# HyeontaeSung/CC-MPC

Measured on AMD Instinct MI355X. Metric: MPC constraint-gen cycles/sec @20Hz (np=5000, ph=8); ellipsoid ΔF-norm vs ref, higher is better.
Workload: dtype f64; 1 GPU; C2: 1 scene x 4 OVs, np=5000/OV, ph=8, Minkowski/MVOE constraint-gen cycle (moments + all (cell,t,tau) half-spaces), one ccmpc_minkowski_cycle launch per step, particles resident in HBM; scenes_per_gpu=1, O=4, N_per_ov=5000, T=8, cells=9, halfspaces_per_cycle=252

## Files before the change

### cc-mpc_amd/csrc/constraints.hpp

```cpp
#pragma once
#include "ccmpc_common.hpp"

namespace ccmpc {


struct M2 {
  double a, b, c, d;
};

__device__ __forceinline__ M2 mul(const M2 &x, const M2 &y) {
  return {x.a * y.a + x.b * y.c, x.a * y.b + x.b * y.d, x.c * y.a + x.d * y.c,
          x.c * y.b + x.d * y.d};
}
__device__ __forceinline__ M2 scale(const M2 &x, double s) {
  return {x.a * s, x.b * s, x.c * s, x.d * s};
}
__device__ __forceinline__ M2 sub(const M2 &x, const M2 &y) {
  return {x.a - y.a, x.b - y.b, x.c - y.c, x.d - y.d};
}
__device__ __forceinline__ M2 add(const M2 &x, const M2 &y) {
  return {x.a + y.a, x.b + y.b, x.c + y.c, x.d + y.d};
}
__device__ __forceinline__ M2 transpose(const M2 &x) { return {x.a, x.c, x.b, x.d}; }

// ... 158 lines not shown
  static constexpr uint64_t start_word() {
    uint64_t x = 0;
    for (int t = 1; t < TC && t < 8; ++t) x |= static_cast<uint64_t>(t * (t - 1) / 2) << (8 * t);
    return x;
  }
};
template <int TC>
__device__ __forceinline__ void pair_of_tc(int p, int &t, int &tau) {
  if constexpr (PairTable<TC>::kFits) {
    constexpr uint64_t lo = PairTable<TC>::t_word(0), hi = PairTable<TC>::t_word(1);
    constexpr uint64_t start = PairTable<TC>::start_word();
    t = static_cast<int>(((p < 16 ? lo : hi) >> (4 * (p & 15))) & 15);
    tau = p - static_cast<int>((start >> (8 * t)) & 255);
  } else {
    pair_of(p, t, tau);
  }
}


static_assert(sizeof(ccmpc_halfspace) == 128, "record size");
static_assert(offsetof(ccmpc_halfspace, d) == 16 && offsetof(ccmpc_halfspace, q01) == 32 &&
                  offsetof(ccmpc_halfspace, r00) == 48 && offsetof(ccmpc_halfspace, r11) == 64 &&
                  offsetof(ccmpc_halfspace, mean0) == 96 && offsetof(ccmpc_halfspace, which) == 112,
              "16-byte field pairs of ccmpc_halfspace");
__device__ __forceinline__ void store_pair(double *p, double a, double b) {
  *reinterpret_cast<double2 *>(p) = make_double2(a, b);
}

struct MinkParams {
  const double *ref_traj;
  const int32_t *cell_ref;
  const double *cell_risk;
  double R, tol;
  int maxiter;
  ccmpc_halfspace *out_rec;
  double *out_prob_lower;
};

struct PairMoments {
  M2 c_t, cov_mu, cov_infer;
  bool ok;
};

struct BlockInverse {
  M2 inv;
  bool ok;
};
__device__ __forceinline__ BlockInverse block_inverse(const M2 &c_tau) {
  BlockInverse bi;
  bi.ok = inv2(c_tau, bi.inv);
  return bi;
}

__device__ __forceinline__ PairMoments pair_moments(const double *C, int rows, int t, int tau) {
  PairMoments pm;
  const BlockInverse bi = block_inverse(block(C, rows, tau, tau));
  pm.c_t = block(C, rows, t, t);
  const M2 c_x = block(C, rows, t, tau);
  const M2 c_xT = block(C, rows, tau, t);
  pm.ok = bi.ok;
  pm.cov_mu = mul(mul(c_x, bi.inv), c_xT);
  pm.cov_infer = sub(pm.c_t, pm.cov_mu);
  return pm;
}

__device__ __forceinline__ double pair_lower_bound(const PairMoments &pm, double gamma) {
  const double root_t = sqrt(fro(pm.c_t));
  const double al = sqrt(fro(pm.cov_infer)) / root_t;
  const double be = sqrt(fro(pm.cov_mu)) / root_t;
  const double x = gamma * (1.0 - al) / be;
  return -expm1(-0.5 * (x * x));
}

__device__ __forceinline__ double pair_scale(const PairMoments &pm, double chi_p, double gamma) {
  const double root_t = sqrt(fro(pm.c_t));
  const double alpha = sqrt(fro(pm.cov_infer)) / root_t;
  const double beta = sqrt(fro(pm.cov_mu)) / root_t;
  const double x = sqrt(chi_p) * beta / gamma + alpha;
  return x * x;
}

__device__ __forceinline__ int closest_tangent(const M2 &S, double c, double n0, double n1,
                                               double proj, double nrm, double na, double &d,
                                               int &which) {
  const double sn0 = S.a * n0 + S.b * n1, sn1 = S.c * n0 + S.d * n1;
  const double q = n0 * sn0 + n1 * sn1;
  if (q <= 0.0) {
    d = NAN;
    which = 0;
    return CCMPC_REC_NO_TANGENT;
  }
  const double delta = c * sqrt(q);
  const double d1 = proj + delta, d2 = proj - delta;
  const double dist0 = fabs(na - d1) / nrm, dist1 = fabs(na - d2) / nrm;
  which = (dist1 < dist0) ? 1 : 0;
  d = which ? d2 : d1;
  return 0;
}

struct TangentFrame {
  double m, n0, proj, nrm, na;
};
__device__ __forceinline__ TangentFrame tangent_frame(double m0, double m1, double a0, double a1) {
  TangentFrame f;
  f.m = -(a0 - m0) / (a1 - m1);
  f.n0 = -f.m;
  const double n1 = 1.0;
  f.proj = f.n0 * m0 + n1 * m1;
  f.nrm = sqrt(f.n0 * f.n0 + n1 * n1);
  f.na = f.n0 * a0 + n1 * a1;
  return f;
}

template <int TC = 0>
__device__ void minkowski_pair(const double *C, const double *mu, const double *ref, int rows_arg,
                               int t, int tau, double chi_r, double chi_p, double R, double tol,
                               int maxiter, ccmpc_halfspace *out) {
  const int rows = TC ? 2 * TC : rows_arg;
  const double m0 = mu[2 * t], m1 = mu[2 * t + 1];
  const TangentFrame f = tangent_frame(m0, m1, ref[2 * t], ref[2 * t + 1]);
  const double m = f.m, n0 = f.n0, n1 = 1.0, proj = f.proj, nrm = f.nrm, na = f.na;
  store_pair(&out->n0, n0, n1);
  store_pair(&out->mean0, m0, m1);
  const PairMoments pm = pair_moments(C, rows, t, tau);
  int status = 0;
  double b1 = NAN, b2 = NAN;
  M2 Q = {NAN, NAN, NAN, NAN}, QR = {NAN, NAN, NAN, NAN};
  bool ok = compute_mvoe(scale(pm.cov_infer, chi_r), scale(pm.cov_mu, chi_p), tol, maxiter, b1, Q,
                         pm.ok);
  store_pair(&out->q01, Q.b, Q.d);
  ok = compute_mvoe(Q, M2{R * R, 0.0, 0.0, R * R}, tol, maxiter, b2, QR, ok);
  if (!ok) status = CCMPC_REC_SINGULAR;
  store_pair(&out->r00, QR.a, QR.b);
  store_pair(&out->r11, QR.d, b1);
  out->beta2 = b2;
  double d = NAN;
  int which = 0, side = 0;
  if (!isfinite(m)) {
    if (status == 0) status = CCMPC_REC_NONFINITE;
  } else {
    const int ts = closest_tangent(QR, 1.0, n0, n1, proj, nrm, na, d, which);
    if (ts != 0) {
      if (status == 0) status = ts;
    } else if (isfinite(d)) {
      side = (proj <= d) ? 1 : -1;
    }
  }
  if (status == 0 && !(isfinite(d) && isfinite(Q.a) && isfinite(QR.a) && isfinite(m0)))
    status = CCMPC_REC_NONFINITE;
  store_pair(&out->d, d, Q.a);
  *reinterpret_cast<int4 *>(&out->which) = make_int4(which, side, status, (t << 16) | tau);
}

template <int NTH, int TC = 0>
__device__ void minkowski_cell(const double *C, const double *mu, int T_arg, int cell,
                               const double *ref, double chi_r, double chi_p, double gamma,
                               const MinkParams &mp, double *lb_s, int tid) {
  constexpr int nthreads = NTH;
  const int T = TC ? TC : T_arg;
  const int rows = 2 * T;
  const int P = T * (T - 1) / 2;
  ccmpc_halfspace *rec = mp.out_rec + static_cast<int64_t>(cell) * P;
  const int half = (nthreads >= 128 && P <= nthreads / 2) ? nthreads / 2 : 0;
  if (half && P <= 2 * 64) {
    if (tid < half) {
      if (tid < P) {
        int t, tau;
        pair_of_tc<TC>(tid, t, tau);
        minkowski_pair<TC>(C, mu, ref, rows, t, tau, chi_r, chi_p, mp.R, mp.tol, mp.maxiter,
                           rec + tid);
      }
      return;
    }
    const int lane = tid - half;
    if (lane >= 64) return;
    for (int p = lane; p < P; p += 64) {
      int t, tau;
      pair_of_tc<TC>(p, t, tau);
      const double lb = pair_lower_bound(pair_moments(C, rows, t, tau), gamma);
      lb_s[p] = lb;
      rec[p].lower_bound = lb;
    }
    asm volatile("s_waitcnt lgkmcnt(0)" ::: "memory");
    if (lane < T) {
      double v = 1.0;
      for (int tau = 0; tau < lane; ++tau) v = fmin(v, lb_s[lane * (lane - 1) / 2 + tau]);
      mp.out_prob_lower[static_cast<int64_t>(cell) * T + lane] = v;
    }
    return;
  }
  const bool lb_side = half && tid >= half;
  const int base = lb_side ? tid - half : tid, stride = half ? half : nthreads;
  for (int p = base; p < P; p += stride) {
    int t, tau;
    pair_of_tc<TC>(p, t, tau);
    if (lb_side || !half) {
      const double lb = pair_lower_bound(pair_moments(C, rows, t, tau), gamma);
      lb_s[p] = lb;
      rec[p].lower_bound = lb;
    }
    if (!lb_side)
      minkowski_pair<TC>(C, mu, ref, rows, t, tau, chi_r, chi_p, mp.R, mp.tol, mp.maxiter, rec + p);
  }
  __syncthreads();
  for (int t = tid; t < T; t += nthreads) {
    double v = 1.0;
    for (int tau = 0; tau < t; ++tau) v = fmin(v, lb_s[t * (t - 1) / 2 + tau]);
    mp.out_prob_lower[static_cast<int64_t>(cell) * T + t] = v;
  }
}

template <int NTH>
__device__ void minkowski_cell(const double *C, const double *mu, int T, int cell,
                               const MinkParams &mp, double *lb_s, int tid) {
  const int rsel = mp.cell_ref ? mp.cell_ref[cell] : 0;
  const double *ref = mp.ref_traj + static_cast<int64_t>(rsel) * (2 * T);
  minkowski_cell<NTH>(C, mu, T, cell, ref, mp.cell_risk[3 * cell + 0],
                      mp.cell_risk[3 * cell + 1], mp.cell_risk[3 * cell + 2], mp, lb_s, tid);
}

void launch_minkowski_rows(const double *mean, const double *cov, int T, int n_cells,
                           const MinkParams &mp, hipStream_t s);

}
```

### cc-mpc_amd/csrc/moments.hip

```cpp
#include "ccmpc_common.hpp"

#ifndef CCMPC_PROBE
#define CCMPC_PROBE 0
#endif

#if CCMPC_PROBE & 4
constexpr int kProbeSlots = 8, kProbeMaxWG = 8192;
__device__ unsigned long long g_probe_ts[kProbeMaxWG * kProbeSlots];
__device__ unsigned long long g_probe_stream_end[kProbeMaxWG];
__device__ __forceinline__ unsigned long long &probe_stream_end_lds() {
  __shared__ unsigned long long t;
  return t;
}
#define PROBE_STREAM_END()                                                                     \
  do {                                                                                         \
    if ((threadIdx.x & 63) == 0)                                                               \
      atomicMax(&probe_stream_end_lds(), __builtin_amdgcn_s_memrealtime());                    \
  } while (0)
#define PROBE_TS(k)                                                                            \
  do {                                                                                         \
    if (threadIdx.x == 0 && blockIdx.x < kProbeMaxWG)                                          \
      g_probe_ts[blockIdx.x * kProbeSlots + (k)] = __builtin_amdgcn_s_memrealtime();           \
    if ((k) == 0 && !(CCMPC_PROBE & 16) && threadIdx.x == 0 && blockIdx.x < kProbeMaxWG)       \
      g_probe_ts[blockIdx.x * kProbeSlots + 7] =                                               \
// ... 115 lines not shown
struct LaneVec<P, 4> {
  using type = Quad<P>;
  __device__ static void load(const P *p, type &q) { load_quad(p, q); }
};
template <typename P>
struct LaneVec<P, 2> {
  using type = Pair<P>;
  __device__ static void load(const P *p, type &q) { load_pair(p, q); }
};

template <typename P, int RB, int S, int W>
__device__ __forceinline__ void load_group(typename LaneVec<P, W>::type (&v)[S][RB],
                                           const P *const (&rowp)[RB], int64_t gbase, int64_t p1,
                                           int g) {
  const int64_t qlast = (p1 - 1) & ~int64_t(W - 1);
#pragma unroll
  for (int s = 0; s < S; ++s) {
    const int64_t q = gbase + 4 * W * s + W * g;
    const int64_t qc = q < qlast ? q : qlast;
#pragma unroll
    for (int b = 0; b < RB; ++b) {
#if CCMPC_PROBE & 2
      LaneVec<P, W>::load(rowp[b] + (qc & (W - 1)), v[s][b]);
#else
      LaneVec<P, W>::load(rowp[b] + qc, v[s][b]);
#endif
    }
  }
}

#ifndef CCMPC_SUBSTEP_FENCE
#define CCMPC_SUBSTEP_FENCE 1
#endif
__device__ __forceinline__ void pin_loaded(Quad<double> &q) {
  ccmpc_d2v lo = {q.lo.x, q.lo.y}, hi = {q.hi.x, q.hi.y};
  asm volatile("" : "+v"(lo), "+v"(hi));
  q.lo = make_double2(lo.x, lo.y);
  q.hi = make_double2(hi.x, hi.y);
}
__device__ __forceinline__ void pin_loaded(Quad<float> &q) {
  ccmpc_f4v t = {q.v.x, q.v.y, q.v.z, q.v.w};
  asm volatile("" : "+v"(t));
  q.v = make_float4(t.x, t.y, t.z, t.w);
}
template <typename P>
__device__ __forceinline__ void pin_loaded(Pair<P> &) {}
template <typename P, int RB, int S, int NACC, int W>
__device__ __forceinline__ void mfma_group(const typename LaneVec<P, W>::type (&raw)[S][RB],
                                           const double (&sh)[RB], const bool (&live)[RB],
                                           int64_t gbase, int64_t p1, int g,
                                           d4 (&acc)[NACC][n_tiles(RB)], double (&s1)[RB]) {
#pragma unroll
  for (int s = 0; s < S; ++s) {
    const int64_t q = gbase + 4 * W * s + W * g;
    typename LaneVec<P, W>::type x[RB];
#pragma unroll
    for (int b = 0; b < RB; ++b) x[b] = raw[s][b];
#if CCMPC_SUBSTEP_FENCE
    if (S > 1) {
      __builtin_amdgcn_sched_barrier(0);
#pragma unroll
      for (int b = 0; b < RB; ++b) pin_loaded(x[b]);
    }
#endif
    double v[RB][W];
#pragma unroll
    for (int b = 0; b < RB; ++b)
#pragma unroll
      for (int j = 0; j < W; ++j)
#if CCMPC_PROBE & 32
        v[b][j] = x[b][j] - sh[b];
#elif CCMPC_PROBE & 64
        v[b][j] = x[b][j];
#else
        v[b][j] = (live[b] && q + j < p1) ? x[b][j] - sh[b] : 0.0;
#endif
#pragma unroll
    for (int j = 0; j < W; ++j) {
      const int a = (NACC == 2) ? (j & 1) : 0;
      int t = 0;
#pragma unroll
      for (int bi = 0; bi < RB; ++bi)
#pragma unroll
        for (int bj = bi; bj < RB; ++bj) {
#if CCMPC_PROBE & 1
          acc[a][t][0] += v[bi][j] * v[bj][j];
#else
          acc[a][t] = __builtin_amdgcn_mfma_f64_16x16x4f64(v[bi][j], v[bj][j], acc[a][t], 0, 0, 0);
#endif
          ++t;
        }
    }
#pragma unroll
    for (int b = 0; b < RB; ++b)
      s1[b] += W == 4 ? (v[b][0] + v[b][1]) + (v[b][2 % W] + v[b][3 % W]) : v[b][0] + v[b][1];
  }
}

#ifndef CCMPC_DEFER_ROOT
#define CCMPC_DEFER_ROOT 1
#endif
__host__ __device__ constexpr bool defer_root(int rb, bool mink, bool bal) {
  return CCMPC_DEFER_ROOT && bal && !mink && rb >= 4;
}

struct EpilogueLds {
  double *slab, *shift, *S, *mean, *cov, *lb, *ref;
  int *flag;
};

#ifndef CCMPC_TAIL_LANDED
#define CCMPC_TAIL_LANDED 1
#endif
template <typename Sch, int NTH, bool MINK, bool COV_IN_LDS, bool DEFER, int TC = 0,
          typename Publish>
__device__ __forceinline__ void cell_epilogue(Publish publish, const ItemLoc &loc, int32_t nit,
                                              int T_arg, const TreeLayout &tree,
                                              const double *__restrict__ origin,
                                              double *__restrict__ out_mean,
                                              double *__restrict__ out_cov, const MinkParams &mp,
                                              const EpilogueLds &L) {
  constexpr int E = Sch::E;
  constexpr bool kLastOrder = std::is_same<Sch, Scheme16<1>>::value;
  const int T = TC ? TC : T_arg;
  const int cell = loc.cell, rows = 2 * T;
  const double o0 = origin ? origin[2 * cell] : 0.0, o1 = origin ? origin[2 * cell + 1] : 0.0;
  double *mean = out_mean + static_cast<int64_t>(cell) * rows;
  double *cov = out_cov + static_cast<int64_t>(cell) * rows * rows;
  if (nit == 1) {
    publish(L.slab, true);
    PROBE_TS(3);
    PROBE_TS(4);
  } else {
    publish(tree.slabs[0] + static_cast<int64_t>(loc.first + loc.chunk_idx) * E, false);
    PROBE_TS(3);
    if (DEFER && nit <= kRootFanIn) return;
    const double *root;
    int32_t root_n;
    const bool last = tree_climb<E, NTH>(tree, loc.chunk_idx, nit, loc.first, cell, L.flag,
                                         &root, &root_n);
    PROBE_TS(4);
    if (!last) return;
    gather_root<Sch, NTH, TC, kLastOrder && CCMPC_GATHER_ORDERED != 0>(
        root, root_n, rows, L.slab, L.cov);
    PROBE_GATHERED();
  }
  if (kLastOrder && CCMPC_TAIL_LANDED != 0 && MINK)
    __builtin_amdgcn_s_waitcnt(0x0f70);
  finalize_cell<Sch, NTH, TC>([&](int e) { return double2{L.slab[e], L.slab[e + 1]}; }, loc.cnt,
                              T, L.shift, L.S, o0, o1, mean, cov, L.mean,
                              COV_IN_LDS ? L.cov : nullptr, L.slab + Sch::GRAM);
  PROBE_TS(5);
  if (MINK)
    minkowski_cell<NTH, TC>(COV_IN_LDS ? L.cov : cov, L.mean, T, cell, L.ref, L.ref[rows],
                            L.ref[rows + 1], L.ref[rows + 2], mp, L.lb, threadIdx.x);
  PROBE_TS(6);
}

struct WaveRange {
  int64_t p0, stride, p1, ngroups;
};
template <bool BAL>
__device__ __forceinline__ WaveRange wave_range(int64_t a, int64_t b, int w, int nw, int64_t wq,
                                                int64_t gs) {
  WaveRange r;
  if (BAL) {
    r.p0 = a + static_cast<int64_t>(w) * gs;
    r.stride = nw * gs;
    r.p1 = b;
    r.ngroups = r.p0 < b ? ceil_div(b - r.p0, r.stride) : 0;
  } else {
    r.p0 = a + static_cast<int64_t>(w) * wq;
    r.stride = gs;
    r.p1 = (r.p0 + wq < b) ? r.p0 + wq : b;
    r.ngroups = r.p1 > r.p0 ? ceil_div(r.p1 - r.p0, gs) : 0;
  }
  return r;
}

#ifndef CCMPC_TAIL_LATE
#define CCMPC_TAIL_LATE 1
#endif
__device__ __forceinline__ double prefetch_tail(const MinkParams &mp, const ItemLoc &loc,
                                                int rows) {
#if CCMPC_TAIL_LATE
  const int i = min(static_cast<int>(threadIdx.x), rows + 2);
  const bool ref = i < rows;
  const double *base = ref ? mp.ref_traj : mp.cell_risk;
  const int64_t at =
      ref ? static_cast<int64_t>(loc.ref_sel) * rows + i : int64_t(3 * loc.cell + (i - rows));
  return base[at];
#else
  if (threadIdx.x < rows) return mp.ref_traj[static_cast<int64_t>(loc.ref_sel) * rows + threadIdx.x];
  if (threadIdx.x < rows + 3) return mp.cell_risk[3 * loc.cell + (threadIdx.x - rows)];
  return 0.0;
#endif
}
__device__ __forceinline__ double prefetch_tail_landed(const MinkParams &mp, const ItemLoc &loc,
                                                       int rows) {
  const double v = prefetch_tail(mp, loc, rows);
  __builtin_amdgcn_sched_barrier(0);
  __builtin_amdgcn_s_waitcnt(0x0f70);
  return v;
}

#ifndef CCMPC_T_CONST
#define CCMPC_T_CONST 1
#endif
#ifndef CCMPC_LOCATE_STRAIGHT
#define CCMPC_LOCATE_STRAIGHT 1
#endif
#ifndef CCMPC_SLOT_FRONT
#define CCMPC_SLOT_FRONT 1
#endif
using SlotArg = uint64_t;
inline SlotArg slot_arg(int64_t slot_cap, int64_t ips) {
  const uint64_t magic = (uint64_t(1) << 31) / static_cast<uint64_t>(ips) + 1u;
  return static_cast<uint64_t>(static_cast<uint32_t>(slot_cap)) | (magic << 32);
}
template <bool SLOT>
using OffArg = std::conditional_t<SLOT, SlotArg, const int64_t *__restrict__>;
#ifndef CCMPC_LOADS_FIRST
#define CCMPC_LOADS_FIRST 1
#endif
template <typename P, int RB, bool MINK, bool BAL, int TC = 0, bool SLOT = false>
__global__ __launch_bounds__(Geo<RB>::THREADS,
                             (MINK && RB == 1) ? 3 : Geo<RB>::MIN_WAVES_PER_SIMD)
void moments_kernel(
    const int64_t *__restrict__ cell_cnt, OffArg<SLOT> cell_off,
    const int32_t *__restrict__ cell_ref, const P *__restrict__ pos, int64_t ld, int n_cells,
    int lg_wq, int32_t whole32, int T_arg, const double *__restrict__ origin, TreeLayout tree,
    double *__restrict__ out_mean, double *__restrict__ out_cov, MinkParams mp) {
  using G = Geo<RB>;
  static_assert(TC == 0 || 2 * TC == 16 * RB, "a constant horizon fills its row blocks exactly");
  const int T = TC ? TC : T_arg;
  const int64_t whole = whole32;
  constexpr int NT = n_tiles(RB);
  constexpr int NACC = G::NACC;
  constexpr int D = 16 * RB;
  constexpr int S = G::S;
  constexpr int W = RB >= 4 ? kWBig : 4;
  constexpr int E = slab_doubles(RB);
  constexpr bool COV_IN_LDS = MINK;
  constexpr bool DEFER = defer_root(RB, MINK, BAL);
  constexpr int XCH = combine_xch_doubles(RB, G::NW) > (MINK ? D * D : 0)
                          ? combine_xch_doubles(RB, G::NW) : D * D;
  static_assert(XCH >= gather_part_doubles(E), "xch must hold the root gather's group slabs");
  __shared__ double xch[XCH];
  __shared__ double slab_lds[E];
  __shared__ double shift_lds[D];
  __shared__ double S_lds[D];
  __shared__ double mean_lds[D];
  __shared__ double lb_s[MINK ? 40 * 39 / 2 : 1];
  __shared__ double ref_lds[MINK ? D + 3 : 1];
  __shared__ int flag;

  const int lane = threadIdx.x & 63;
  const int w = __builtin_amdgcn_readfirstlane(threadIdx.x >> 6);
  const int rows = 2 * T;
  const int lg_chunk = lg_wq + lg_waves_per_item(RB);

  auto item = [=](const ItemLoc &loc_in, int32_t nit, int64_t a, int64_t b) {
    const int r = lane & 15;
    const int g = lane >> 4;
    ItemLoc loc = loc_in;
    int64_t cnt = loc.cnt;
    double pre = (MINK && !CCMPC_TAIL_LATE) ? prefetch_tail(mp, loc, rows) : 0.0;
    constexpr int DP = RB >= 3 ? CCMPC_DEPTH_BIG : kDepth;
    constexpr bool FRONT = CCMPC_LOADS_FIRST != 0 && RB == 1 && !BAL;
    double sh[RB];
    d4 acc[NACC][NT];
    double s1[RB];
    if constexpr (FRONT) {
      constexpr int GS = 4 * W * S;
      static_assert(RB == 1 && GS == 64, "the front is written for RB = 1");
      bool rr = b - a > (int64_t(1) << lg_chunk);
      int64_t p0 = a + (rr ? int64_t(w) * GS : int64_t(w) << lg_wq);
      const bool live0 = r < rows;
      int64_t row_at = static_cast<int64_t>(live0 ? r : 0) * ld + loc.off;
      const P *rowp[RB];
      bool live[RB] = {live0};
      typename LaneVec<P, W>::type buf[DP][S][RB];
      int64_t p1, ngroups, st;
      double x0s = 0.0;
      if constexpr (SLOT) {
        const int64_t p0s =
            (static_cast<int64_t>(loc.chunk_idx) << lg_chunk) + (int64_t(w) << lg_wq);
        const int64_t n_ld = cell_cnt[loc.cell];
        __builtin_amdgcn_sched_barrier(0);
        x0s = static_cast<double>(pos[row_at]);
        const P *gb = pos + (row_at + p0s);
#pragma unroll
        for (int s = 0; s < S; ++s) {
#if CCMPC_PROBE & 2
          LaneVec<P, W>::load(pos + row_at + ((W * g) & (W - 1)), buf[0][s][0]);
#else
          LaneVec<P, W>::load(gb + (4 * W * s + W * g), buf[0][s][0]);
#endif
        }
        asm volatile("" ::: "memory");
        __builtin_amdgcn_sched_barrier(0);
        const int32_t *rp = cell_ref ? cell_ref + loc.cell
                                     : reinterpret_cast<const int32_t *>(cell_cnt + loc.cell);
        const int32_t rs_ld = *rp;
        PROBE_TS(1);
        cnt = n_ld;
        loc.cnt = n_ld;
        loc.ref_sel = cell_ref ? rs_ld : 0;
// ... 179 lines not shown
      __builtin_expect(static_cast<unsigned>(n_cells - 1) < 64u, 1)) {
    if (!locate_item_straight(blockIdx.x, cell_cnt, cell_off, n_cells, lg_chunk, loc, cell_ref,
                              whole))
      return;
  } else {
    if (!locate_item(blockIdx.x, cell_cnt, cell_off, n_cells, lg_chunk, loc,
                     cell_ref, whole))
      return;
    if (CCMPC_LOCATE_STRAIGHT != 0 && RB == 1) __builtin_amdgcn_s_waitcnt(0x0f70);
  }
  PROBE_TS(1);
  const int32_t nit = items_of(loc.cnt, lg_chunk, whole);
  const int64_t i0 = static_cast<int64_t>(loc.chunk_idx) << lg_chunk;
  const int64_t i1 = nit == 1 ? loc.cnt : min(i0 + (int64_t(1) << lg_chunk), loc.cnt);
  item(loc, nit, i0, i1);
  }
}

#ifndef CCMPC_F32_WIDE4
#define CCMPC_F32_WIDE4 1
#endif
template <typename P>
struct Row4 {
  using type = Pair<P>;
  static constexpr int W = 2;
  __device__ static void load(const P *p, type &q) { load_pair(p, q); }
};
#if CCMPC_F32_WIDE4
template <>
struct Row4<float> {
  using type = Quad<float>;
  static constexpr int W = 4;
  __device__ static void load(const float *p, type &q) {
    if constexpr (CCMPC_NT_PAIR != 0) {
      const ccmpc_f4v t = __builtin_nontemporal_load(reinterpret_cast<const ccmpc_f4v *>(p));
      q.v = make_float4(t.x, t.y, t.z, t.w);
    } else {
      q.v = *reinterpret_cast<const float4 *>(p);
    }
  }
};
#endif

template <typename P, int NB>
__device__ __forceinline__ void load_group4(typename Row4<P>::type (&v)[NB],
                                            const P *const (&rowp)[NB], int64_t gbase, int64_t p1,
                                            int m) {
  constexpr int W = Row4<P>::W;
  const int64_t qlast = (p1 - 1) & ~int64_t(W - 1);
  const int64_t q = gbase + W * m;
  const int64_t qc = q < qlast ? q : qlast;
#pragma unroll
  for (int I = 0; I < NB; ++I) Row4<P>::load(rowp[I] + qc, v[I]);
}

#ifndef CCMPC_ROWLOAD4
#define CCMPC_ROWLOAD4 0
#endif
__device__ __forceinline__ double bperm_f64(int addr, double x) {
  const uint64_t u = __builtin_bit_cast(uint64_t, x);
  const uint32_t lo = static_cast<uint32_t>(
      __builtin_amdgcn_ds_bpermute(addr, static_cast<int>(static_cast<uint32_t>(u))));
  const uint32_t hi = static_cast<uint32_t>(
      __builtin_amdgcn_ds_bpermute(addr, static_cast<int>(static_cast<uint32_t>(u >> 32))));
  return __builtin_bit_cast(double, (static_cast<uint64_t>(hi) << 32) | lo);
}
__device__ __forceinline__ float bperm_f32(int addr, float x) {
  return __builtin_bit_cast(
      float, __builtin_amdgcn_ds_bpermute(addr, __builtin_bit_cast(int, x)));
}
__device__ __forceinline__ Pair<double> bperm_pair(int addr, const Pair<double> &p) {
  Pair<double> r;
  r.v.x = bperm_f64(addr, p.v.x);
  r.v.y = bperm_f64(addr, p.v.y);
  return r;
}
__device__ __forceinline__ Pair<float> bperm_pair(int addr, const Pair<float> &p) {
  Pair<float> r;
  r.v.x = bperm_f32(addr, p.v.x);
  r.v.y = bperm_f32(addr, p.v.y);
  return r;
}

template <typename P, int NB>
__device__ __forceinline__ void mfma_group4(const typename Row4<P>::type (&loaded)[NB],
                                            const double (&sh)[NB], const bool (&live)[NB],
                                            int64_t gbase, int64_t p1, int m, int paddr,
                                            double (&acc)[n_pairs(NB)], double (&s1)[NB]) {
  constexpr int W = Row4<P>::W;
  const int64_t q = gbase + W * m;
#if CCMPC_ROWLOAD4
  static_assert(W == 2, "CCMPC_ROWLOAD4 is the pair layout");
  Pair<P> raw[NB];
#pragma unroll
  for (int I = 0; I < NB; ++I) raw[I] = bperm_pair(paddr, loaded[I]);
#else
  const typename Row4<P>::type(&raw)[NB] = loaded;
  (void)paddr;
#endif
#pragma unroll
  for (int j = 0; j < W; ++j) {
    double v[NB];
#pragma unroll
    for (int I = 0; I < NB; ++I) {
#if CCMPC_PROBE & 32
      v[I] = raw[I][j] - sh[I];
#elif CCMPC_PROBE & 64
      v[I] = raw[I][j];
#else
      v[I] = (live[I] && q + j < p1) ? raw[I][j] - sh[I] : 0.0;
#endif
      s1[I] += v[I];
    }
    int p = 0;
#pragma unroll
    for (int I = 0; I < NB; ++I)
#pragma unroll
      for (int J = I; J < NB; ++J) {
        acc[p] = __builtin_amdgcn_mfma_f64_4x4x4f64(v[I], v[J], acc[p], 0, 0, 0);
        ++p;
      }
  }
}

#ifndef CCMPC_NW4
#define CCMPC_NW4 4
#endif
constexpr int kNW4 = CCMPC_NW4;
constexpr int kThreads4 = kNW4 * 64;
#ifndef CCMPC_M4_OCC
#define CCMPC_M4_OCC(NB) (((NB) <= 5 ? 3 : 2) * 4 / kNW4 > 0 ? ((NB) <= 5 ? 3 : 2) * 4 / kNW4 : 1)
#endif
#ifndef CCMPC_M4_OCC_F32
#define CCMPC_M4_OCC_F32 0
#endif
template <typename P>
constexpr int m4_occ(int nb) {
  return std::is_same_v<P, float> && CCMPC_M4_OCC_F32 > 0 ? CCMPC_M4_OCC_F32 : CCMPC_M4_OCC(nb);
}

template <typename P, int NB, bool MINK, bool BAL>
__global__ __launch_bounds__(kThreads4, m4_occ<P>(NB)) void moments4_kernel(
    const int64_t *__restrict__ cell_cnt, const int64_t *__restrict__ cell_off,
    const int32_t *__restrict__ cell_ref, const P *__restrict__ pos, int64_t ld, int n_cells,
    int lg_wq, int T, const double *__restrict__ origin, TreeLayout tree,
    double *__restrict__ out_mean, double *__restrict__ out_cov, MinkParams mp) {
  using Sch = Scheme4<NB>;
  constexpr int NP = Sch::NP, D = Sch::D, E = Sch::E;
  __shared__ double xch[kNW4 * Combine4Layout<NB>::XS];
  __shared__ double slab_lds[E];
  __shared__ double shift_lds[D];
  __shared__ double S_lds[D];
  __shared__ double mean_lds[D];
  __shared__ double lb_s[MINK ? 12 * 11 / 2 : 1];
  __shared__ double ref_lds[MINK ? D + 3 : 1];
  __shared__ int flag;

  const int lane = threadIdx.x & 63;
  const int w = __builtin_amdgcn_readfirstlane(threadIdx.x >> 6);
  const int rows = 2 * T;
  const int lg_chunk = lg_wq + 2;

  auto item = [=](const ItemLoc &loc, int32_t nit, int64_t a, int64_t b) {
    const int c = lane & 3, m = lane >> 2;
#if CCMPC_ROWLOAD4
    const int rl = lane >> 4, ml = lane & 15;
#else
    const int rl = c, ml = m;
#endif
    const int paddr = 4 * (16 * c + m);
    const int64_t cnt = loc.cnt;
    double pre = (MINK && !CCMPC_TAIL_LATE) ? prefetch_tail(mp, loc, rows) : 0.0;
    const WaveRange wr = wave_range<BAL>(a, b, w, kNW4, int64_t(1) << lg_wq, 16 * Row4<P>::W);
    const int64_t p1 = wr.p1;

    double sh[NB];
    const P *rowp[NB];
    bool live[NB];
#pragma unroll
    for (int I = 0; I < NB; ++I) {
      const int R = 4 * I + c, RL = 4 * I + rl;
      live[I] = R < rows;
      rowp[I] = pos + static_cast<int64_t>(RL < rows ? RL : 0) * ld + loc.off;
      sh[I] = (live[I] && cnt > 0)
                  ? static_cast<double>(pos[static_cast<int64_t>(R) * ld + loc.off]) : 0.0;
    }
    double acc[NP];
#pragma unroll
    for (int p = 0; p < NP; ++p) acc[p] = 0.0;
    double s1[NB];
#pragma unroll
    for (int I = 0; I < NB; ++I) s1[I] = 0.0;

    const int64_t ngroups = wr.ngroups, st = wr.stride;
    constexpr int DP = BAL ? (std::is_same_v<P, float> ? kDepth4BalF32 : kDepth4Bal) : kDepth4;
    typename Row4<P>::type buf[DP][NB];
    if (ngroups > 0) {
#pragma unroll
      for (int d = 0; d < DP - 1; ++d) load_group4<P, NB>(buf[d], rowp, wr.p0 + d * st, p1, ml);
      if (MINK && CCMPC_TAIL_LATE) {
        __builtin_amdgcn_sched_barrier(0);
        pre = prefetch_tail(mp, loc, rows);
      }
      int64_t gi = 0;
      for (; gi + DP <= ngroups; gi += DP) {
        if (BAL) progress_prio(gi, ngroups);
#pragma unroll
        for (int d = 0; d < DP; ++d) {
          load_group4<P, NB>(buf[(d + DP - 1) % DP], rowp, wr.p0 + (gi + d + DP - 1) * st, p1, ml);
          __builtin_amdgcn_sched_barrier(0);
          mfma_group4<P, NB>(buf[d], sh, live, wr.p0 + (gi + d) * st, p1, m, paddr, acc, s1);
          __builtin_amdgcn_sched_barrier(0);
        }
      }
#pragma unroll
      for (int d = 0; d < DP - 1; ++d)
        if (gi + d < ngroups)
          mfma_group4<P, NB>(buf[d], sh, live, wr.p0 + (gi + d) * st, p1, m, paddr, acc, s1);
    } else if (MINK && CCMPC_TAIL_LATE) {
      pre = prefetch_tail_landed(mp, loc, rows);
    }
    PROBE_TS(2);
    PROBE_STREAM_END();
#if CCMPC_PROGRESS_PRIO
    __builtin_amdgcn_s_setprio(0);
#endif

    if (MINK && threadIdx.x < rows + 3) ref_lds[threadIdx.x] = pre;
#pragma unroll
    for (int I = 0; I < NB; ++I)
      if (w == 0 && m == 0) shift_lds[4 * I + c] = sh[I];
    static_assert(kNW4 * Combine4Layout<NB>::XS >= D * D, "xch must hold the covariance");
    static_assert(kNW4 * Combine4Layout<NB>::XS >= gather_part_doubles(E),
                  "xch must hold the root gather's group slabs");
    const EpilogueLds L{slab_lds, shift_lds, S_lds, mean_lds, xch, lb_s, ref_lds, &flag};
    cell_epilogue<Sch, kThreads4, MINK, MINK, false>(
        [&](double *dst, bool to_lds) { combine4<NB, kNW4>(acc, s1, xch, dst, to_lds); }, loc,
        nit, T, tree, origin, out_mean, out_cov, mp, L);
  };

  PROBE_TS(0);
  if (BAL) {
    ItemLoc loc;
    int64_t chunk;
    if (!locate_balanced(blockIdx.x, gridDim.x, cell_cnt, cell_off, n_cells, loc, &chunk,
                         cell_ref))
      return;
    PROBE_TS(1);
    const int64_t i0 = static_cast<int64_t>(loc.chunk_idx) * chunk;
    item(loc, static_cast<int32_t>(loc.cnt > 0 ? ceil_div_fast(loc.cnt, chunk) : 1), i0,
         min(i0 + chunk, loc.cnt));
    return;
  }
  ItemLoc loc;
  if (!locate_item(blockIdx.x, cell_cnt, cell_off, n_cells, lg_chunk, loc,
                   cell_ref))
    return;
  PROBE_TS(1);
  const int64_t i0 = static_cast<int64_t>(loc.chunk_idx) << lg_chunk;
  const int64_t i1 = min(i0 + (int64_t(1) << lg_chunk), loc.cnt);
  item(loc, items_of(loc.cnt, lg_chunk), i0, i1);
}

__device__ __forceinline__ void cell_items_balanced(int cell, int G, const int64_t *__restrict__ cnt,
                                                    int n_cells, int32_t &first, int32_t &nit,
                                                    int64_t &n) {
  const int lane = threadIdx.x & 63;
  double part = 0.0;
  for (int base = 0; base < n_cells; base += 64)
    part += base + lane < n_cells ? static_cast<double>(cnt[base + lane]) : 0.0;
  const double td = wave_sum_dpp_f64(part);
  const int64_t n0 = lane < n_cells ? cnt[lane] : 0, n1 = lane + 64 < n_cells ? cnt[lane + 64] : 0;
  const int64_t chunk = balanced_chunk(td, G, n_cells, n0, n1);
  int32_t before = 0;
  first = 0;
  nit = 0;
  n = 0;
  for (int base = 0; base < n_cells; base += 64) {
    const int c = base + lane;
    const int64_t nn = c < n_cells ? cnt[c] : 0;
    const int32_t mine =
        c < n_cells ? static_cast<int32_t>(nn > 0 ? ceil_div_fast(nn, chunk) : 1) : 0;
    const int32_t incl = wave_incl_scan_i32(mine);
    if (cell < base + 64) {
      const int l = cell - base;
      first = before + lane_i32(incl - mine, l);
      nit = lane_i32(mine, l);
      n = lane_i64(nn, l);
      return;
    }
    before += lane_i32(incl, 63);
  }
}

constexpr int kRootGroups = kRootFanIn / kFanIn;
static_assert(kRootGroups * kFanIn == kRootFanIn, "root = whole fan-in groups");
template <int RB>
struct RootGeo {
  static constexpr int D = 16 * RB;
  static constexpr int PAIRS = 128 + D / 2;
  static constexpr int GATHER = kRootGroups * PAIRS;
  static constexpr int THREADS = (GATHER + D + 63) / 64 * 64;
  static_assert(THREADS <= 1024, "deferred root: kRootFanIn too wide for one workgroup");
  static_assert(sizeof(double2) * kRootGroups * PAIRS + 2 * sizeof(double) * D <= 64 * 1024,
                "deferred root: LDS partials exceed the static 64 KiB");
};
template <typename P, int RB>
// ... 391 lines not shown
```

Measured before the change: 138,500 cycles/s.

## Split Minkowski pair tail across chain and helper waves via LDS handoff

Splits each (t,tau) pair's Minkowski half-space computation so that one wave runs the serial MVOE chain while a second wave computes the tangent frame, validity flags and part of the output record in parallel. The helper passes its results through enlarged LDS, a barrier joins the two, and the chain thread finishes the closest-tangent step. Any pair that fails the fast path falls back to the full per-pair routine. The goal is to shorten the critical path of the per-cell tail, at the cost of an extra __syncthreads, more LDS, and some pair moments computed twice.

```diff
diff --git a/cc-mpc_amd/csrc/constraints.hpp b/cc-mpc_amd/csrc/constraints.hpp
--- a/cc-mpc_amd/csrc/constraints.hpp
+++ b/cc-mpc_amd/csrc/constraints.hpp
@@ -334,7 +334,74 @@
   *reinterpret_cast<int4 *>(&out->which) = make_int4(which, side, status, (t << 16) | tau);
 }
 
-template <int NTH, int TC = 0>
+#ifndef CCMPC_TAIL_SPLIT
+#define CCMPC_TAIL_SPLIT 1
+#endif
+
+constexpr int kTailSplitMaxPairs = 64, kTailSplitFields = 5;
+constexpr int kTailSplitLds = kTailSplitMaxPairs * (1 + kTailSplitFields);
+
+__device__ __forceinline__ void tail_helper(const PairMoments &pm, const double *mu,
+                                            const double *ref, int t, double chi_r,
+                                            ccmpc_halfspace *out, double *fr) {
+  const double m0 = mu[2 * t], m1 = mu[2 * t + 1];
+  const TangentFrame f = tangent_frame(m0, m1, ref[2 * t], ref[2 * t + 1]);
+  store_pair(&out->n0, f.n0, 1.0);
+  store_pair(&out->mean0, m0, m1);
+  const bool ok = pm.ok && lu_ok(scale(pm.cov_infer, chi_r)) && isfinite(f.m) && isfinite(m0);
+  fr[0 * kTailSplitMaxPairs] = f.n0;
+  fr[1 * kTailSplitMaxPairs] = f.proj;
+  fr[2 * kTailSplitMaxPairs] = f.nrm;
+  fr[3 * kTailSplitMaxPairs] = f.na;
+  fr[4 * kTailSplitMaxPairs] = ok ? 1.0 : 0.0;
+}
+
+struct TailChain {
+  M2 QR;
+  double Qa;
+  bool q_ok;
+};
+template <int TC>
+__device__ __forceinline__ TailChain tail_chain(const double *C, int rows_arg, int t, int tau,
+                                                double chi_r, double chi_p, double R, double tol,
+                                                int maxiter, ccmpc_halfspace *out) {
+  const int rows = TC ? 2 * TC : rows_arg;
+  const PairMoments pm = pair_moments(C, rows, t, tau);
+  const M2 S1 = scale(pm.cov_infer, chi_r), S2 = scale(pm.cov_mu, chi_p);
+  const MvoeChain c1 = mvoe_chain(S1, S2, tol, maxiter);
+  const M2 Q = add(scale(S1, 1.0 + rcp_nr(c1.beta)), scale(S2, 1.0 + c1.beta));
+  store_pair(&out->q01, Q.b, Q.d);
+  const M2 RR = {R * R, 0.0, 0.0, R * R};
+  const MvoeChain c2 = mvoe_chain(Q, RR, tol, maxiter);
+  TailChain r;
+  r.QR = add(scale(Q, 1.0 + rcp_nr(c2.beta)), scale(RR, 1.0 + c2.beta));
+  r.Qa = Q.a;
+  r.q_ok = c2.ok;
+  store_pair(&out->r00, r.QR.a, r.QR.b);
+  store_pair(&out->r11, r.QR.d, c1.beta);
+  out->beta2 = c2.beta;
+  return r;
+}
+
+__device__ __forceinline__ bool tail_finish(const TailChain &r, const double *fr, int t, int tau,
+                                            ccmpc_halfspace *out) {
+  const double n0 = fr[0 * kTailSplitMaxPairs], proj = fr[1 * kTailSplitMaxPairs];
+  const double nrm = fr[2 * kTailSplitMaxPairs], na = fr[3 * kTailSplitMaxPairs];
+  const bool flags = fr[4 * kTailSplitMaxPairs] != 0.0;
+  double d = NAN;
+  int which = 0;
+  const int ts = closest_tangent(r.QR, 1.0, n0, 1.0, proj, nrm, na, d, which);
+  const bool regular =
+      flags && r.q_ok && ts == 0 && isfinite(d) && isfinite(r.Qa) && isfinite(r.QR.a);
+  if (regular) {
+    const int side = (proj <= d) ? 1 : -1;
+    store_pair(&out->d, d, r.Qa);
+    *reinterpret_cast<int4 *>(&out->which) = make_int4(which, side, 0, (t << 16) | tau);
+  }
+  return regular;
+}
+
+template <int NTH, int TC = 0, bool SPLIT = false>
 __device__ void minkowski_cell(const double *C, const double *mu, int T_arg, int cell,
                                const double *ref, double chi_r, double chi_p, double gamma,
                                const MinkParams &mp, double *lb_s, int tid) {
@@ -344,6 +411,45 @@
   const int P = T * (T - 1) / 2;
   ccmpc_halfspace *rec = mp.out_rec + static_cast<int64_t>(cell) * P;
   const int half = (nthreads >= 128 && P <= nthreads / 2) ? nthreads / 2 : 0;
+  if constexpr (SPLIT) {
+    if (half >= 128 && P <= kTailSplitMaxPairs) {
+      const bool chain = tid < P;
+      const bool helper = tid >= 64 && tid < 64 + P;
+      const int lane = tid - half;
+      const bool lower = lane >= 0 && lane < P;
+      const int p = chain ? tid : (helper ? tid - 64 : lane);
+      double *fr = lb_s + kTailSplitMaxPairs + p;
+      int t = 0, tau = 0;
+      TailChain tc;
+      if (chain | helper | lower) pair_of_tc<TC>(p, t, tau);
+      if (chain) {
+        tc = tail_chain<TC>(C, rows, t, tau, chi_r, chi_p, mp.R, mp.tol, mp.maxiter, rec + p);
+      } else if (helper) {
+        tail_helper(pair_moments(C, rows, t, tau), mu, ref, t, chi_r, rec + p, fr);
+      } else if (lower) {
+        const double lb = pair_lower_bound(pair_moments(C, rows, t, tau), gamma);
+        lb_s[p] = lb;
+        rec[p].lower_bound = lb;
+      }
+#if defined(CCMPC_PROBE) && (CCMPC_PROBE & 128)
+      if (chain) tail_finish(tc, fr, t, tau, rec + p);
+#else
+      __syncthreads();
+      if (chain && __builtin_expect(!tail_finish(tc, fr, t, tau, rec + p), 0))
+        minkowski_pair<TC>(C, mu, ref, rows, t, tau, chi_r, chi_p, mp.R, mp.tol, mp.maxiter,
+                           rec + p);
+#endif
+      if (lane >= 0 && lane < 64) {
+        asm volatile("s_waitcnt lgkmcnt(0)" ::: "memory");
+        if (lane < T) {
+          double v = 1.0;
+          for (int k = 0; k < lane; ++k) v = fmin(v, lb_s[lane * (lane - 1) / 2 + k]);
+          mp.out_prob_lower[static_cast<int64_t>(cell) * T + lane] = v;
+        }
+      }
+      return;
+    }
+  }
   if (half && P <= 2 * 64) {
     if (tid < half) {
       if (tid < P) {
diff --git a/cc-mpc_amd/csrc/moments.hip b/cc-mpc_amd/csrc/moments.hip
--- a/cc-mpc_amd/csrc/moments.hip
+++ b/cc-mpc_amd/csrc/moments.hip
@@ -291,8 +291,9 @@
                               COV_IN_LDS ? L.cov : nullptr, L.slab + Sch::GRAM);
   PROBE_TS(5);
   if (MINK)
-    minkowski_cell<NTH, TC>(COV_IN_LDS ? L.cov : cov, L.mean, T, cell, L.ref, L.ref[rows],
-                            L.ref[rows + 1], L.ref[rows + 2], mp, L.lb, threadIdx.x);
+    minkowski_cell<NTH, TC, CCMPC_TAIL_SPLIT != 0>(COV_IN_LDS ? L.cov : cov, L.mean, T, cell, L.ref,
+                                                   L.ref[rows], L.ref[rows + 1], L.ref[rows + 2],
+                                                   mp, L.lb, threadIdx.x);
   PROBE_TS(6);
 }
 
@@ -778,7 +779,7 @@
   __shared__ double shift_lds[D];
   __shared__ double S_lds[D];
   __shared__ double mean_lds[D];
-  __shared__ double lb_s[MINK ? 12 * 11 / 2 : 1];
+  __shared__ double lb_s[MINK ? (CCMPC_TAIL_SPLIT != 0 ? kTailSplitLds : 12 * 11 / 2) : 1];
   __shared__ double ref_lds[MINK ? D + 3 : 1];
   __shared__ int flag;
 
```

New measurement: 138,900 cycles/s (median of 6 runs). About the same (+0.3%).
